# yyamamoto79/guetzli-cuda-opencl

Measured on AMD Instinct MI355X. Metric: Mpixels/s end-to-end encode @ q=95; achieved HBM GB/s on Butteraugli pass, higher is better.
Workload: dtype f32

## Files before the change

### guetzli-cuda-opencl_amd/csrc/kernels/gz_device.hip

```cpp
#include <hip/hip_runtime.h>

#include <math.h>
#include <stdio.h>
#include <string.h>
#include <time.h>

#include <algorithm>
#include <chrono>
#include <atomic>
#include <list>
#include <map>
#include <condition_variable>
#include <mutex>
#include <tuple>
#include <string>
#include <vector>

#include "../runtime/engine.h"
#include "../host/thread_pool.h"
#include "gz_math.h"

namespace gz {
__constant__ GzTables c_tab;
}
// ... 223 lines not shown
  do {                                                 \
    hipError_t e_ = (call);                            \
    if (e_ != hipSuccess) return Fail(#call, (int)e_); \
  } while (0)
#define GZ_LAUNCH()                                               \
  do {                                                            \
    hipError_t e_ = hipGetLastError();                            \
    if (e_ != hipSuccess) return Fail("kernel launch", (int)e_);  \
  } while (0)

namespace {
std::atomic<int> g_prof_on{0};
std::mutex g_prof_mu;
std::map<std::string, std::pair<long, double>> g_prof;
}

void ProfileEnable(bool on) { g_prof_on.store(on ? 1 : 0); }
void ProfileReset() {
  std::lock_guard<std::mutex> lk(g_prof_mu);
  g_prof.clear();
}
bool ProfileGet(const char* name, long* count, double* total_ms) {
  std::lock_guard<std::mutex> lk(g_prof_mu);
  auto it = g_prof.find(name);
  if (it == g_prof.end()) return false;
  *count = it->second.first;
  *total_ms = it->second.second;
  return true;
}
std::string ProfileNames() {
  std::lock_guard<std::mutex> lk(g_prof_mu);
  std::string out;
  for (auto& kv : g_prof) {
    if (!out.empty()) out += ",";
    out += kv.first;
  }
  return out;
}

void Engine::ProfBegin(const char* name) {
  if (!g_prof_on.load()) return;
  hipEvent_t a = nullptr, b = nullptr;
  if (hipEventCreate(&a) != hipSuccess || hipEventCreate(&b) != hipSuccess) return;
  hipEventRecord(a, static_cast<hipStream_t>(stream_));
  pending_.push_back({name, a, b});
}
void Engine::ProfEnd() {
  if (pending_.empty() || !g_prof_on.load()) return;
  hipEventRecord(static_cast<hipEvent_t>(pending_.back().stop), static_cast<hipStream_t>(stream_));
}
void Engine::ProfMark(const char* name) {
  if (!g_prof_on.load()) return;
  for (auto it = pending_.rbegin(); it != pending_.rend(); ++it)
    if (it->name == name) {
      hipEventRecord(static_cast<hipEvent_t>(it->stop), static_cast<hipStream_t>(stream_));
      return;
    }
}

void Engine::ProfFlush() {
  if (pending_.empty()) return;
  std::lock_guard<std::mutex> lk(g_prof_mu);
  for (auto& p : pending_) {
    float ms = 0.0f;
    if (hipEventSynchronize(static_cast<hipEvent_t>(p.stop)) == hipSuccess &&
        hipEventElapsedTime(&ms, static_cast<hipEvent_t>(p.start), static_cast<hipEvent_t>(p.stop)) == hipSuccess) {
      auto& e = g_prof[p.name];
      e.first += 1;
      e.second += ms;
    }
    hipEventDestroy(static_cast<hipEvent_t>(p.start));
    hipEventDestroy(static_cast<hipEvent_t>(p.stop));
  }
  pending_.clear();
}

#define GZ_TIMED(name, ...) \
  do {                      \
    ProfBegin(name);        \
    __VA_ARGS__;            \
    ProfEnd();              \
    GZ_LAUNCH();            \
  } while (0)

bool Engine::Fail(const char* what, int code) {
  char buf[256];
  snprintf(buf, sizeof(buf), "%s failed: %s (%d)", what,
           hipGetErrorString(static_cast<hipError_t>(code)), code);
  err_ = buf;
  failed_ = true;
  return false;
}

std::unique_ptr<Engine> Engine::Create(int device, int w, int h, std::string* err) {
  std::unique_ptr<Engine> e(new Engine);
  auto fail = [&](const std::string& m) {
    if (err) *err = m;
    return std::unique_ptr<Engine>();
  };
  if (w < 8 || h < 8 || w >= (1 << 16) || h >= (1 << 16)) return fail("unsupported image size");
  int ndev = 0;
  if (hipGetDeviceCount(&ndev) != hipSuccess || ndev == 0) return fail("no HIP device available");
  if (device < 0 || device >= ndev || device >= 64) return fail("bad device index");
  if (hipSetDevice(device) != hipSuccess) return fail("hipSetDevice failed");
  {
    std::lock_guard<std::mutex> lk(g_tab_mu);
    if (!g_tab_uploaded[device]) {
      const GzTables& t = HostTables();
      for (const BlurSpec& b : t.blur)
        if ((kBlurTile - 1) * b.step + 2 * b.radius + 1 + b.step > kBlurLds || 2 * b.radius + 1 > kMaxTaps ||
            b.step < 1 || b.step > 4)
          return fail("blur spec exceeds the tiled kernel's LDS span");
      for (int sig = 0; sig < kNumSigmas; ++sig)
        if (t.blur[sig].step != kBlurGeomStep[sig] || t.blur[sig].radius != kBlurGeomR[sig])
          return fail("blur geometry differs from the compiled BlurGeom table");
      for (int sig = kSigEdgeX; sig <= kSigEdgeB; ++sig)
        if (t.blur[sig].step != 1 || t.blur[sig].radius > kB2MaxR)
          return fail("edge blur spec does not fit the fused 2-D kernel");
      if (hipMemcpyToSymbol(HIP_SYMBOL(c_tab), &t, sizeof(t)) != hipSuccess)
        return fail("table upload failed");
      g_tab_uploaded[device] = true;
    }
  }
  e->device_ = device;
  e->w_ = w;
  e->h_ = h;
  e->bw_ = (w + 7) / 8;
  e->bh_ = (h + 7) / 8;
  e->nb_ = e->bw_ * e->bh_;
  e->rw_ = (w + 2) / 3;
  e->rh_ = (h + 2) / 3;
  e->n_ = static_cast<size_t>(w) * h;
  hipStream_t s;
  if (hipStreamCreateWithFlags(&s, hipStreamNonBlocking) != hipSuccess) return fail("stream");
  e->stream_ = s;
  const size_t n = e->n_, rn = static_cast<size_t>(e->rw_) * e->rh_;
  const size_t nc = static_cast<size_t>(e->nb_) * 64 * 3;
  bool ok = true;
  auto alloc = [&](void** p, size_t bytes) {
    if (ok && hipMalloc(p, bytes) != hipSuccess) ok = false;
    e->bytes_ += bytes;
  };
  alloc(reinterpret_cast<void**>(&e->d_rgb_), 3 * n);
  alloc(reinterpret_cast<void**>(&e->d_orig_), nc * sizeof(int16_t));
  alloc(reinterpret_cast<void**>(&e->d_cur_), nc * sizeof(int16_t));
  alloc(reinterpret_cast<void**>(&e->d_ref_xyb_), 3 * n * 4);
  alloc(reinterpret_cast<void**>(&e->d_lin_), 3 * n * 4);
  alloc(reinterpret_cast<void**>(&e->d_px8_), n * 4);
  alloc(reinterpret_cast<void**>(&e->d_xyb_), 3 * n * 4);
  alloc(reinterpret_cast<void**>(&e->d_m0_), 3 * n * 4);
  alloc(reinterpret_cast<void**>(&e->d_m1_), 3 * n * 4);
  alloc(reinterpret_cast<void**>(&e->d_tmp_), 6 * n * 4);
  alloc(reinterpret_cast<void**>(&e->d_bl_), 6 * n * 4);
  alloc(reinterpret_cast<void**>(&e->d_ma_), 3 * n * 4);
  alloc(reinterpret_cast<void**>(&e->d_mb_), 3 * n * 4);
  alloc(reinterpret_cast<void**>(&e->d_edge_), 3 * rn * 4);
  alloc(reinterpret_cast<void**>(&e->d_dc_), 3 * rn * 4);
  alloc(reinterpret_cast<void**>(&e->d_ac_), 3 * rn * 4);
  alloc(reinterpret_cast<void**>(&e->d_resval_), rn * 4);
  alloc(reinterpret_cast<void**>(&e->d_block_max_), e->nb_ * 4);
  alloc(reinterpret_cast<void**>(&e->d_mask_scale_), 3 * e->nb_ * 4);
  alloc(&e->d_zero_out_, static_cast<size_t>(e->nb_) * 192 * sizeof(CoeffData));
  alloc(reinterpret_cast<void**>(&e->d_zero_count_), static_cast<size_t>(e->nb_) * 4);
  alloc(reinterpret_cast<void**>(&e->d_zero_order_), static_cast<size_t>(e->nb_) * 4);
  alloc(reinterpret_cast<void**>(&e->d_zero_off_), static_cast<size_t>(e->nb_ + 1) * 4);
  alloc(reinterpret_cast<void**>(&e->d_zero_nnz_), static_cast<size_t>(e->nb_) * 4);
// ... 835 lines not shown
  }
  GZ_HIP(hipMemsetAsync(static_cast<char*>(d_ord_) + L.mbe, 0, static_cast<size_t>(nb_) * 4, s));
  GZ_HIP(hipMemsetAsync(static_cast<char*>(d_ord_) + L.sel, 0, L.cnt8 - L.sel, s));
  ord_adv_dir_ = 0;
  ord_n_ = 0;
  return true;
}

bool Engine::OrderEntriesCapacity(size_t n) {
  const size_t bytes = n * sizeof(OrderEntry);
  if (bytes > d_ord_entries_cap_) {
    if (d_ord_entries_) GZ_HIP(hipFree(d_ord_entries_));
    d_ord_entries_ = nullptr;
    d_ord_entries_cap_ = 0;
    const size_t cap = bytes + bytes / 4 + 4096;
    GZ_HIP(hipMalloc(&d_ord_entries_, cap));
    d_ord_entries_cap_ = cap;
  }
  return true;
}

bool Engine::OrderBuild(int direction, int rblock, double target_distance, bool zero_bmax,
                        const std::vector<int>& last_indexes, size_t* n_entries, int* blocks_to_change,
                        float floor_limit, int64_t* below_floor) {
  hipStream_t s = static_cast<hipStream_t>(stream_);
  GZ_HIP(hipSetDevice(device_));
  if (ord_cand_n_ < 0 || !d_ord_) return Fail("OrderBuild without candidates", 0);
  const size_t max_entries = static_cast<size_t>(ord_cand_n_) + static_cast<size_t>(nb_);
  if (!OrderEntriesCapacity(max_entries)) return false;
  if (static_cast<int>(last_indexes.size()) != nb_ || rblock < 1 || rblock > 4)
    return Fail("OrderBuild arguments", 0);
  const OrdLayout L(nb_);
  char* base = static_cast<char*>(d_ord_);
  uint32_t* sel = reinterpret_cast<uint32_t*>(base + L.sel);
  int adv_dir = 0;
  if (rblock == 1) {
    uint8_t* l8 = reinterpret_cast<uint8_t*>(h_ord_);
    int bad = 0;
    for (int b = 0; b < nb_; ++b) {
      bad |= last_indexes[b] & ~0xff;
      l8[b] = static_cast<uint8_t>(last_indexes[b]);
    }
    if (bad) return Fail("OrderBuild: last index above 255", 0);
    adv_dir = ord_adv_dir_;
    ord_adv_dir_ = 0;
  }
  ord_h1_ ^= 1;
  BuildArgs g;
  g.bmax = d_block_max_;
  g.zero_bmax = zero_bmax ? 1 : 0;
  g.bw = bw_;
  g.bh = bh_;
  g.r = rblock;
  g.direction = direction;
  g.td = target_distance;
  g.weight = reinterpret_cast<float*>(base + L.weight);
  g.active = reinterpret_cast<const int*>(base + L.active);
  g.mbe = reinterpret_cast<float*>(base + L.mbe);
  g.adv_vt = ord_adv_vt_;
  g.adv_dir = adv_dir;
  g.copy_last = rblock == 1 ? 1 : 0;
  g.last = reinterpret_cast<int*>(base + L.last);
  g.last_host = reinterpret_cast<const uint8_t*>(m_ord_);
  g.off = d_zero_off_;
  g.cand_n = ord_cand_n_;
  g.cand_err = d_cand_err_;
  g.out = static_cast<OrderEntry*>(d_ord_entries_);
  g.h1 = sel + SelLayout::h1 + ord_h1_ * kSelBins;
  g.h1_next = sel + SelLayout::h1 + (ord_h1_ ^ 1) * kSelBins;
  SelState* st = reinterpret_cast<SelState*>(sel + SelLayout::state);
  g.reserve = &st->reserve[ord_h1_];
  g.reserve_next = &st->reserve[ord_h1_ ^ 1];
  const unsigned groups = static_cast<unsigned>((nb_ + kBuildBlocks - 1) / kBuildBlocks);
  g.wg_host = m_ord_ + nb_ + kOrdInfoInts + 16 + static_cast<int>((sizeof(SelHost) + 63) / 64 * 16);
  const int* wg = h_ord_ + nb_ + kOrdInfoInts + 16 + static_cast<int>((sizeof(SelHost) + 63) / 64 * 16);
  g.floor_limit = floor_limit;
  g.blo = ord_lo_;
  g.bhi = std::min(ord_hi_, nb_);
  ord_h1_summed_ = false;
  if (direction < 0 && (rblock > 1 || !GZ_FUSE_ACTIVE))
    GZ_TIMED("order_build", k_order_active<<<static_cast<unsigned>((nb_ + 255) / 256), 256, 0, s>>>(
                                d_block_max_, zero_bmax ? 1 : 0, bw_, bh_, rblock, target_distance,
                                reinterpret_cast<int*>(base + L.active)));
  GZ_TIMED("order_build", k_order_build<<<groups, 256, 0, s>>>(g));
  GZ_HIP(WaitOnStream(s));
  ProfFlush();
  long long tot[3] = {0, 0, 0};
  for (unsigned k = 0; k < groups; ++k)
    for (int x = 0; x < 3; ++x) tot[x] += wg[4 * k + x];
  *blocks_to_change = static_cast<int>(tot[1]);
  *n_entries = static_cast<size_t>(tot[0]);
  if (below_floor) *below_floor = tot[2];
  ord_n_ = *n_entries;
  return true;
}

bool Engine::OrderFetch(std::pair<int, float>* out, size_t n) {
  static_assert(sizeof(OrderEntry) == sizeof(std::pair<int, float>), "entry layout");
  hipStream_t s = static_cast<hipStream_t>(stream_);
  GZ_HIP(hipSetDevice(device_));
  if (!n) return true;
  if (n != ord_n_) return Fail("OrderFetch entry count", 0);
  const size_t bytes = n * sizeof(OrderEntry);
  if (bytes > h_ord_entries_cap_) {
    if (h_ord_entries_) GZ_HIP(hipHostFree(h_ord_entries_));
    h_ord_entries_ = nullptr;
    h_ord_entries_cap_ = 0;
    const size_t cap = bytes + bytes / 4 + 4096;
    GZ_HIP(hipHostMalloc(&h_ord_entries_, cap));
    h_ord_entries_cap_ = cap;
  }
  GZ_HIP(hipMemcpyAsync(h_ord_entries_, d_ord_entries_, bytes, hipMemcpyDeviceToHost, s));
  GZ_HIP(WaitIdle(s));
  ProfFlush();
  const auto* src = static_cast<const std::pair<int, float>*>(h_ord_entries_);
  const int* wg = h_ord_ + nb_ + kOrdInfoInts + 16 + static_cast<int>((sizeof(SelHost) + 63) / 64 * 16);
  const int groups = (nb_ + kBuildBlocks - 1) / kBuildBlocks;
  size_t at = 0;
  for (int g = 0; g < groups; ++g) {
    const int cnt = wg[4 * g], base = wg[4 * g + 3];
    if (cnt == 0) continue;
    if (cnt < 0 || base < 0 || static_cast<size_t>(base) + cnt > n || at + cnt > n)
      return Fail("OrderFetch: workgroup ranges", 0);
    memcpy(static_cast<void*>(out + at), src + base, static_cast<size_t>(cnt) * sizeof(OrderEntry));
    at += static_cast<size_t>(cnt);
  }
  if (at != n) return Fail("OrderFetch: entry count", 0);
  return true;
}

bool Engine::BulkCountsStaging() {
  if (h_bulk_) return true;
  void* h = nullptr;
  void* m = nullptr;
  if (hipHostMalloc(&h, static_cast<size_t>(nb_) + 64, hipHostMallocCoherent) != hipSuccess) {
    return Fail("BulkApply: pinned allocation failed", 0);
  }
  if (hipHostGetDevicePointer(&m, h, 0) != hipSuccess) {
    (void)hipHostFree(h);
    return Fail("BulkApply: mapped address", 0);
  }
  h_bulk_ = static_cast<uint8_t*>(h);
  m_bulk_ = static_cast<uint8_t*>(m);
  bytes_ += static_cast<size_t>(nb_) + 64;
  return true;
}

bool Engine::BulkApplyEnqueue(int direction, const int quant[3][64], const uint8_t* cnt_dev, const uint32_t* sel,
                              const uint8_t* last8, uint8_t* cnt_host) {
  hipStream_t s = static_cast<hipStream_t>(stream_);
  const OrdLayout L(nb_);
  QuantMatrix qm;
  memcpy(qm.q, quant, sizeof(qm.q));
  JpegQuantF qf;
  for (int c = 0; c < 3; ++c)
    for (int k = 0; k < 64; ++k) qf.qz[c][k] = static_cast<float>(quant[c][c_natural_order[k]]);
  const size_t stage_groups = (3 * static_cast<size_t>(nb_) + kStageBlocks - 1) / kStageBlocks;
  const unsigned groups = static_cast<unsigned>(
      std::min(stage_groups, (static_cast<size_t>(nb_) + kBulkWaves - 1) / kBulkWaves));
  GZ_TIMED("bulk_apply", k_bulk_apply<<<groups, kBulkThreads, 0, s>>>(
      cnt_dev, reinterpret_cast<const int*>(static_cast<char*>(d_ord_) + L.last), d_zero_off_, ord_cand_n_,
      d_cand_idx_, nb_, direction, d_orig_, qm, qf, d_cur_, d_jhist_, sel, last8, cnt_host),
      k_hist_fold<<<1, 1024, 0, s>>>(d_jhist_, m_jhist_, 0));
  return true;
}

bool Engine::BulkApply(int direction, const int quant[3][64], const uint8_t* cnt, int32_t delta[3][256],
                       const std::vector<int>* last_indexes) {
  hipStream_t s = static_cast<hipStream_t>(stream_);
  GZ_HIP(hipSetDevice(device_));
  if (last_indexes && !d_ord_ && !OrderReset()) return false;
  if (ord_cand_n_ < 0 || !d_ord_) return Fail("BulkApply without a change order", 0);
  if (!BulkCountsStaging()) return false;
  memcpy(h_bulk_, cnt, static_cast<size_t>(nb_));
  const uint8_t* last8 = nullptr;
  if (last_indexes) {
    if (static_cast<int>(last_indexes->size()) != nb_) return Fail("BulkApply: last indexes", 0);
    uint8_t* l8 = reinterpret_cast<uint8_t*>(h_ord_);
    int bad = 0;
    for (int b = 0; b < nb_; ++b) {
      bad |= (*last_indexes)[b] & ~0xff;
      l8[b] = static_cast<uint8_t>((*last_indexes)[b]);
    }
    if (bad) return Fail("BulkApply: last index above 255", 0);
    last8 = reinterpret_cast<const uint8_t*>(m_ord_);
  }
  if (!BulkApplyEnqueue(direction, quant, m_bulk_, nullptr, last8, nullptr)) return false;
  GZ_HIP(WaitOnStream(s));
  ProfFlush();
  for (int c = 0; c < 3; ++c)
    for (int i = 0; i < 256; ++i) delta[c][i] = static_cast<int32_t>(h_jhist_[(2 * c + 1) * 256 + i]);
  return true;
}

static size_t SelCollectLds(int cap) {
  return 2 * static_cast<size_t>(cap) * sizeof(unsigned long long) + (kSelSortBins + 1) * sizeof(uint32_t);
}

bool Engine::OrderSelect(size_t bulk, size_t window, int direction, const int quant[3][64], bool apply,
                         OrderSelection* out, int32_t delta[3][256]) {
  hipStream_t s = static_cast<hipStream_t>(stream_);
  GZ_HIP(hipSetDevice(device_));
  if (ord_cand_n_ < 0 || !d_ord_) return Fail("OrderSelect without a change order", 0);
  const size_t n = ord_n_;
  if ((ord_x_ ? ord_frame_n_ : n) == 0 || bulk >= (ord_x_ ? ord_frame_n_ : n) || window == 0)
    return Fail("OrderSelect arguments", 0);
  if (!BulkCountsStaging()) return false;
  window = std::min<size_t>(window, kSelCandMax / 2);
  if (!h_win_) {
    GZ_HIP(hipHostMalloc(&h_win_, kSelCandMax * sizeof(OrderEntry), hipHostMallocCoherent));
    GZ_HIP(hipHostGetDevicePointer(&m_win_, h_win_, 0));
    GZ_HIP(hipMalloc(&d_win_, kSelCandMax * sizeof(unsigned long long)));
    bytes_ += kSelCandMax * sizeof(unsigned long long);
    GZ_HIP(hipFuncSetAttribute(reinterpret_cast<const void*>(k_sel_finish),
                               hipFuncAttributeMaxDynamicSharedMemorySize,
                               static_cast<int>(SelCollectLds(kSelCandMax))));
  }
  int cap = 1024;
  while (static_cast<size_t>(cap) < 2 * window && cap < kSelCandMax) cap <<= 1;
  const OrdLayout L(nb_);
  char* base = static_cast<char*>(d_ord_);
  uint32_t* sel = reinterpret_cast<uint32_t*>(base + L.sel);
  uint8_t* cnt8 = reinterpret_cast<uint8_t*>(base + L.cnt8);
  const OrderEntry* e = static_cast<const OrderEntry*>(d_ord_entries_);
  const int has_prefix = bulk > 0 ? 1 : 0;
  const size_t fn = ord_x_ ? ord_frame_n_ : n;
  const long long ta = static_cast<long long>(bulk) - 1;
  const long long tb = static_cast<long long>(std::min(fn - 1, bulk + window - 1));
  SelHost* host = reinterpret_cast<SelHost*>(h_ord_ + nb_ + kOrdInfoInts + 16);
  SelHost* mhost = reinterpret_cast<SelHost*>(m_ord_ + nb_ + kOrdInfoInts + 16);
  host->done = 0;
  static const int force_open = getenv("GZ_SELECT_OPEN") ? atoi(getenv("GZ_SELECT_OPEN")) : 0;
  const size_t chunks = (n + 1023) / 1024;
  const unsigned rgroups = static_cast<unsigned>(std::max<size_t>(1, std::min<size_t>(512, chunks)));
  static const size_t cmax = getenv("GZ_SEL_CGROUPS") ? static_cast<size_t>(atoi(getenv("GZ_SEL_CGROUPS"))) : 512;
  const unsigned cgroups = static_cast<unsigned>(std::max<size_t>(1, std::min<size_t>(cmax, chunks)));
  uint32_t* h1 = sel + SelLayout::h1 + ord_h1_ * kSelBins;
  const int blo = ord_x_ ? ord_lo_ : 0, bhi = ord_x_ ? std::min(ord_hi_, nb_) : nb_;
  const int gbase = ord_x_ ? ord_gbase_ : 0;
  if (!ord_x_) {
    GZ_TIMED("order_select",
             (k_sel_refine<<<rgroups, 256, 0, s>>>(e, static_cast<int>(n), has_prefix, ta, tb, h1, sel,
                                                    reinterpret_cast<uint32_t*>(cnt8), (nb_ + 3) / 4),
              k_sel_collect<<<cgroups, kSelThreads, 0, s>>>(e, static_cast<int>(n), has_prefix,
                                                             static_cast<long long>(bulk), ta, tb, sel,
                                                             reinterpret_cast<uint32_t*>(cnt8),
// ... 344 lines not shown
```

### guetzli-cuda-opencl_amd/csrc/kernels/jpeg_kernels.inc

```
#pragma once

namespace gz {

struct JpegQuantF {
  float qz[3][64];
};

constexpr int kJDcSyms = 17;
struct JpegCodesArg {
  uint8_t dc[3][kJDcSyms][3];
  uint8_t ac[3][256][3];
};

constexpr int c_natural_order[64] = {
    0,  1,  8,  16, 9,  2,  3,  10, 17, 24, 32, 25, 18, 11, 4,  5,  12, 19, 26, 33, 40, 48,
    41, 34, 27, 20, 13, 6,  7,  14, 21, 28, 35, 42, 49, 56, 57, 50, 43, 36, 29, 22, 15, 23,
    30, 37, 44, 51, 58, 59, 52, 45, 38, 31, 39, 46, 53, 60, 61, 54, 47, 55, 62, 63,
};

__device__ __forceinline__ int log2_floor_nz(uint32_t v) { return 31 - __clz(v); }

__device__ __forceinline__ int16_t jpeg_quant(int16_t v, float q) {
  return static_cast<int16_t>(static_cast<int>(static_cast<float>(v) / q));
}

__device__ __forceinline__ int16_t jpeg_quant_rcp(int16_t v, int q, float rq) {
  const int a = v < 0 ? -static_cast<int>(v) : static_cast<int>(v);
  int n = static_cast<int>(static_cast<float>(a) * rq);
  n -= n * q > a ? 1 : 0;
  n += (n + 1) * q <= a ? 1 : 0;
  return static_cast<int16_t>(v < 0 ? -n : n);
}

__device__ __forceinline__ int16_t jpeg_dc(const int16_t* __restrict__ cur, const JpegQuantF& q,
                                           int nb, int c, int b) {
  if (b < 0) return 0;
  return jpeg_quant(cur[(static_cast<size_t>(c) * nb + b) * 64], q.qz[c][0]);
}

constexpr int kJHistCopies = 8;
__global__ __launch_bounds__(1024) void k_hist_fold(uint32_t* __restrict__ hist, uint32_t* __restrict__ host_out,
                                                    int chroma) {
  for (int i = threadIdx.x; i < 6 * 256; i += 1024) {
    uint32_t v = 0;
#pragma unroll
    for (int k = 0; k < kJHistCopies; ++k) {
      v += hist[k * (6 * 256) + i];
      hist[k * (6 * 256) + i] = 0u;
    }
    host_out[i] = v;
  }
  if (chroma && threadIdx.x == 0) {
    unsigned long long* chroma_nz = reinterpret_cast<unsigned long long*>(hist + kJHistCopies * 6 * 256);
    unsigned long long cn = 0;
    for (int k = 0; k < kJHistCopies; ++k) {
      cn += chroma_nz[k];
      chroma_nz[k] = 0ull;
    }
    host_out[6 * 256] = static_cast<uint32_t>(cn);
    host_out[6 * 256 + 1] = static_cast<uint32_t>(cn >> 32);
  }
}
__host__ __device__ constexpr size_t jhist_device_bytes(size_t stage_groups) {
  return kJHistCopies * 6 * 256 * 4 + kJHistCopies * 8 + (2 + stage_groups / 64 + 1) * 4;
}
constexpr int kStageBlocks = 256;
constexpr int kStageThreads = 4 * kStageBlocks;
constexpr int kStageStride = 33;

template <int kQuarter>
__device__ __forceinline__ void jpeg_stage_quarter(const uint32_t* __restrict__ sb, int c,
                                                   const JpegQuantF& q, int16_t z[16], uint32_t* m16,
                                                   int* nz_stored) {
  const int16_t* v = reinterpret_cast<const int16_t*>(sb);
  uint32_t m = 0;
  int nz = 0;
#pragma unroll
  for (int i = 0; i < 16; ++i) {
    const int k = 16 * kQuarter + i;
    const int16_t sv = v[c_natural_order[k]];
    nz += sv != 0;
    z[i] = jpeg_quant(sv, q.qz[c][k]);
    m |= static_cast<uint32_t>(z[i] != 0) << i;
  }
  *m16 = m;
  *nz_stored = nz;
}

template <int kQuarter>
__device__ __forceinline__ void jpeg_stage_symbols(const int16_t z[16], uint64_t m64,
                                                   uint32_t* __restrict__ hac) {
#pragma unroll
  for (int i = 0; i < 16; ++i) {
    const int k = 16 * kQuarter + i;
    if (k == 0 || z[i] == 0) continue;
    const uint64_t below = m64 & ~1ull & ((1ull << k) - 1);
    const int prev = below ? 63 - __clzll(below) : 0;
    const int run = k - prev - 1;
    if (run > 15) atomicAdd(&hac[0xf0], static_cast<uint32_t>(run >> 4));
    const int a = z[i] < 0 ? -z[i] : z[i];
    atomicAdd(&hac[((run & 15) << 4) + log2_floor_nz(a) + 1], 1u);
  }
}

__global__ __launch_bounds__(kStageThreads) void k_jpeg_stage(const int16_t* __restrict__ cur, JpegQuantF q,
                                                     int nb, int m0, int m1,
                                                     uint32_t* __restrict__ hist) {
  unsigned long long* chroma_nz = reinterpret_cast<unsigned long long*>(hist + kJHistCopies * 6 * 256);
  __shared__ uint32_t lh_all[4][6 * 256];
  __shared__ uint32_t sblk[kStageBlocks * kStageStride];
  __shared__ uint16_t smask[kStageBlocks][4];
  __shared__ int nz_red[kStageThreads / 64];
  const int tid = threadIdx.x, lane = tid & 63, wv = tid >> 6;
  for (int i = tid; i < 4 * 6 * 256; i += kStageThreads) (&lh_all[0][0])[i] = 0;
  const int nr = m1 - m0;
  const int ntot = 3 * nr;
  const int t0 = blockIdx.x * kStageBlocks;
  {
#pragma unroll
    for (int r = 0; r < 2; ++r) {
      const int j = tid + kStageThreads * r;
      const int lb = j >> 3, part = j & 7;
      if (t0 + lb < ntot) {
        const int tt = t0 + lb, cc = tt / nr;
        const uint4 u = reinterpret_cast<const uint4*>(
            cur + (static_cast<size_t>(cc) * nb + m0 + (tt - cc * nr)) * 64)[part];
        uint32_t* d = &sblk[lb * kStageStride + 4 * part];
        d[0] = u.x;
        d[1] = u.y;
        d[2] = u.z;
        d[3] = u.w;
      }
    }
  }
  __syncthreads();
  const int quarter = wv & 3;
  const int lb = 64 * (wv >> 2) + lane;
  const bool on = t0 + lb < ntot;
  const int c = on ? (t0 + lb) / nr : 0;
  const int t = c * nb + m0 + (t0 + lb - c * nr);
  int16_t z[16];
  uint32_t m16 = 0;
  int nz_stored = 0;
  if (on) {
// ... 435 lines not shown
      s_tail = v;
    } else {
      words[fw + i - wbase] = v;
      ff += count_ff_bytes(v, nbytes);
    }
  }
  ff = wave_sum_i(ff);
  if (lane == 0) s_ff[wv] = ff;
  __syncthreads();
  if (tid == 0) {
    int f = s_ff[0] + s_ff[1] + s_ff[2] + s_ff[3];
    const bool one = nw == 1;
    if (head_shared) {
      if (t == 0) {
        host[kCodeHostFirst] = s_head;
      } else {
        const uint64_t info = (one && tail_shared) ? 8u : static_cast<uint64_t>(one ? end_bytes : 4);
        code_store(&side[2 * t], (info << 32) | s_head);
        asm volatile("s_waitcnt vmcnt(0)" ::: "memory");
        if (atomicAdd(&seam[t], 1u) == 1u) {
          asm volatile("" ::: "memory");
          atomicExch(&seam[t], 0u);
          const uint32_t v = static_cast<uint32_t>(code_load(&side[2 * t - 1])) | s_head;
          if (info & 8u) {
            host[kCodeHostLast] = v;
          } else {
            words[fw - wbase] = v;
            f += count_ff_bytes(v, static_cast<int>(info));
          }
        }
      }
    }
    if (tail_shared && !(one && head_shared)) {
      if (last_wg) {
        host[kCodeHostLast] = s_tail;
      } else {
        code_store(&side[2 * t + 1], static_cast<uint64_t>(s_tail));
        asm volatile("s_waitcnt vmcnt(0)" ::: "memory");
        if (atomicAdd(&seam[t + 1], 1u) == 1u) {
          asm volatile("" ::: "memory");
          atomicExch(&seam[t + 1], 0u);
          const uint64_t h = code_load(&side[2 * (t + 1)]);
          const uint32_t v = static_cast<uint32_t>(h) | s_tail;
          const uint32_t info = static_cast<uint32_t>(h >> 32);
          if (info & 8u) {
            host[kCodeHostLast] = v;
          } else {
            words[lwd - wbase] = v;
            f += count_ff_bytes(v, static_cast<int>(info));
          }
        }
      }
    }
    host[kCodeHostFf + t] = static_cast<uint32_t>(f);
    if (last_wg) {
      const unsigned long long total = E - base;
      host[kCodeHostBits] = static_cast<uint32_t>(total);
      host[kCodeHostBits + 1] = static_cast<uint32_t>(total >> 32);
    }
  }
}


constexpr int kBulkThreads = 1024;
constexpr int kBulkWaves = kBulkThreads / 64;

__device__ __forceinline__ void bulk_symbols(int16_t z, int lane, uint32_t* h, uint32_t w) {
  const uint64_t m = __ballot(z != 0) & ~1ull;
  if (lane > 0 && z != 0) {
    const uint64_t below = m & ((1ull << lane) - 1);
    const int prev = below ? 63 - __clzll(below) : 0;
    const int run = lane - prev - 1;
    if (run > 15) atomicAdd(&h[0xf0], w * static_cast<uint32_t>(run >> 4));
    const int a = z < 0 ? -z : z;
    atomicAdd(&h[((run & 15) << 4) + log2_floor_nz(a) + 1], w);
  }
  if (lane == 63 && !(m >> 63)) atomicAdd(&h[0], w);
}

__global__ __launch_bounds__(kBulkThreads) void k_bulk_apply(
    const uint8_t* __restrict__ cnt, const int* __restrict__ last, const int* __restrict__ off, int cand_n,
    const uint8_t* __restrict__ cand_idx, int nb, int direction, const int16_t* __restrict__ orig,
    const QuantMatrix qm, const JpegQuantF q, int16_t* __restrict__ cur, uint32_t* __restrict__ hist,
    const uint32_t* __restrict__ sel, const uint8_t* __restrict__ last8, uint8_t* __restrict__ cnt_host) {
  if (sel && reinterpret_cast<const SelState*>(sel + SelLayout::state)->open) return;
  __shared__ uint32_t lh[3 * 256];
  __shared__ float lq[3 * 64];
  __shared__ int lqm[3 * 64];
  __shared__ uint8_t lchg[kBulkWaves][3 * 64];
  const int tid = threadIdx.x, lane = tid & 63, wv = wave_id();
  for (int i = tid; i < 3 * 256; i += kBulkThreads) lh[i] = 0;
  if (tid < 3 * 64) {
    lq[tid] = reinterpret_cast<const float*>(&q)[tid];
    lqm[tid] = reinterpret_cast<const int*>(&qm)[tid];
  }
  __syncthreads();
  const int nat = c_natural_order[lane];
  uint8_t* chg = lchg[wv];
  const int back = direction < 0 ? -1 : 0;
  const int nw = static_cast<int>(gridDim.x) * kBulkWaves;
  const int w = static_cast<int>(blockIdx.x) * kBulkWaves + wv;
  for (int b0 = w; b0 < nb; b0 += 64 * nw) {
    const int bl = b0 + lane * nw;
    const int my_n = bl < nb ? cnt[bl] : 0;
    if (cnt_host && bl < nb) cnt_host[bl] = static_cast<uint8_t>(my_n);
    const int my_off = my_n ? max(0, min(off[bl], cand_n - 1)) : 0;
    const int my_li = my_n ? (last8 ? static_cast<int>(last8[bl]) : last[bl]) : 0;
    uint64_t todo = __ballot(my_n != 0);
    while (todo) {
      const int j = __builtin_ctzll(todo);
      todo &= todo - 1;
      const int b = b0 + j * nw;
      const int n = __builtin_amdgcn_readlane(my_n, j);
      const int first = __builtin_amdgcn_readlane(my_off, j) + __builtin_amdgcn_readlane(my_li, j) + back;
      int16_t v[3];
#pragma unroll
      for (int c = 0; c < 3; ++c) v[c] = cur[(static_cast<size_t>(c) * nb + b) * 64 + nat];
      int ci[3];
#pragma unroll
      for (int r = 0; r < 3; ++r) ci[r] = lane + 64 * r < n ? cand_idx[first + (lane + 64 * r) * direction] : -1;
      chg[lane] = 0;
      chg[64 + lane] = 0;
      chg[128 + lane] = 0;
      asm volatile("s_waitcnt lgkmcnt(0)" ::: "memory");
#pragma unroll
      for (int r = 0; r < 3; ++r)
        if (ci[r] >= 0) chg[ci[r]] = 1;
      asm volatile("s_waitcnt lgkmcnt(0)" ::: "memory");
#pragma unroll
      for (int c = 0; c < 3; ++c) {
        const bool ch = chg[64 * c + nat] != 0;
        if (!__ballot(ch)) continue;
        const size_t e = (static_cast<size_t>(c) * nb + b) * 64 + nat;
        int16_t nv = v[c];
        if (ch) {
          nv = direction > 0 ? static_cast<int16_t>(0) : quantize_coeff(orig[e], lqm[64 * c + nat]);
          cur[e] = nv;
        }
        const float qq = lq[64 * c + lane];
        const int16_t z0 = jpeg_quant(v[c], qq), z1 = jpeg_quant(nv, qq);
        if (!__ballot(z0 != z1)) continue;
        bulk_symbols(z0, lane, &lh[256 * c], ~0u);
        bulk_symbols(z1, lane, &lh[256 * c], 1u);
      }
    }
  }
  __syncthreads();
  uint32_t* hcopy = hist + (blockIdx.x % kJHistCopies) * (6 * 256);
  for (int i = tid; i < 3 * 256; i += kBulkThreads) {
    const uint32_t v = lh[i];
    if (v) atomicAdd(&hcopy[(2 * (i >> 8) + 1) * 256 + (i & 255)], v);
  }
}

}
```

### guetzli-cuda-opencl_amd/csrc/kernels/order_kernels.inc

```
#pragma once

namespace gz {

__device__ __forceinline__ float order_max(float a, float b) { return a < b ? b : a; }

__device__ __forceinline__ void order_range(const int* __restrict__ off, int cand_n, int b, int* offset,
                                            int* num) {
  *offset = max(0, min(off[b], cand_n - 1));
  *num = off[b + 1] - *offset;
}

__device__ __forceinline__ float order_local_max(const float* __restrict__ bmax, int zero_bmax, int bw, int bh,
                                                 int bx, int by, int r, float tdf) {
  float m = tdf;
  for (int y = max(0, by - r); y < min(bh, by + 1 + r); ++y) {
    float rm = tdf;
    for (int x = max(0, bx - r); x < min(bw, bx + 1 + r); ++x) rm = order_max(rm, zero_bmax ? 0.0f : bmax[y * bw + x]);
    m = order_max(m, rm);
  }
  return m;
}
__global__ __launch_bounds__(256) void k_order_active(const float* __restrict__ bmax, int zero_bmax, int bw, int bh,
                                                      int r, double td, int* __restrict__ active) {
  const int b = blockIdx.x * 256 + threadIdx.x;
// ... 51 lines not shown
  const int t = threadIdx.x, lane = t & 63, wv = t >> 6;
  uint32_t v[2][per];
  int loc[2] = {0, 0};
#pragma unroll
  for (int x = 0; x < 2; ++x) {
    const uint4* p = reinterpret_cast<const uint4*>((x ? hb : ha) + t * per);
#pragma unroll
    for (int q = 0; q < per / 4; ++q) {
      const uint4 u = p[q];
      v[x][4 * q] = u.x;
      v[x][4 * q + 1] = u.y;
      v[x][4 * q + 2] = u.z;
      v[x][4 * q + 3] = u.w;
    }
#pragma unroll
    for (int k = 0; k < per; ++k) loc[x] += static_cast<int>(v[x][k]);
  }
  int inc[2] = {loc[0], loc[1]};
#pragma unroll
  for (int d = 1; d < 64; d <<= 1) {
#pragma unroll
    for (int x = 0; x < 2; ++x) {
      const int o = __shfl_up(inc[x], d, 64);
      if (lane >= d) inc[x] += o;
    }
  }
  if (lane == 63) {
    s_w[0][wv] = inc[0];
    s_w[1][wv] = inc[1];
  }
  if (t == 0) {
    s_res.j[0] = kSelBins - 1;
    s_res.below[0] = base_a;
    s_res.eq[0] = 0;
    s_res.j[1] = kSelBins - 1;
    s_res.below[1] = base_b;
    s_res.eq[1] = 0;
  }
  __syncthreads();
#pragma unroll
  for (int x = 0; x < 2; ++x) {
    if (x == 0 && !want_a) continue;
    int pre = 0;
    for (int k = 0; k < wv; ++k) pre += s_w[x][k];
    const long long target = x ? tb : ta;
    long long cum = static_cast<long long>(x ? base_b : base_a) + pre + inc[x] - loc[x];
    const bool last = t == NT - 1;
    if ((cum <= target && cum + loc[x] > target) || (last && cum + loc[x] <= target)) {
      int j = t * per + per - 1;
      int eq = static_cast<int>(v[x][per - 1]);
      long long below = cum + loc[x] - eq;
#pragma unroll
      for (int k = 0; k < per; ++k) {
        if (cum + v[x][k] > target) {
          j = t * per + k;
          below = cum;
          eq = static_cast<int>(v[x][k]);
          break;
        }
        cum += v[x][k];
      }
      s_res.j[x] = j;
      s_res.below[x] = static_cast<int>(below);
      s_res.eq[x] = eq;
    }
  }
  __syncthreads();
  *res = s_res;
  __syncthreads();
}

struct OrderEntry {
  int block;
  float key;
};
#ifndef GZ_FUSE_ACTIVE
#define GZ_FUSE_ACTIVE 1
#endif
#ifndef GZ_BUILD_BLOCKS
#define GZ_BUILD_BLOCKS 128
#endif
constexpr int kBuildBlocks = GZ_BUILD_BLOCKS;
static_assert(kBuildBlocks <= 256 && 256 % kBuildBlocks == 0, "blocks per build workgroup");
struct BuildArgs {
  const float* bmax;
  int zero_bmax, bw, bh, r, direction;
  double td;
  float* weight;
  const int* active;
  float* mbe;
  float adv_vt;
  int adv_dir;
  int copy_last;
  int* last;
  const uint8_t* last_host;
  const int* off;
  int cand_n;
  const float* cand_err;
  OrderEntry* out;
  uint32_t* h1;
  uint32_t* h1_next;
  int* reserve;
  int* reserve_next;
  int* wg_host;
  float floor_limit;
  int blo, bhi;
};
__global__ __launch_bounds__(256) void k_order_build(BuildArgs g) {
  __shared__ int s_off[256 + 1];
  __shared__ int s_last[kBuildBlocks], s_cand[kBuildBlocks];
  __shared__ float s_w[kBuildBlocks], s_mbe[kBuildBlocks];
  __shared__ uint32_t s_h[kSelBins];
  __shared__ int s_base, s_with, s_below;
  __shared__ int s_wsum[4], s_wwith[4];
  const int t = threadIdx.x, lane = t & 63, wv = t >> 6;
  const int nb = g.bw * g.bh;
  const int b0 = static_cast<int>(blockIdx.x) * kBuildBlocks;
  for (int k = static_cast<int>(blockIdx.x) * 256 + t; k < kSelBins; k += static_cast<int>(gridDim.x) * 256)
    g.h1_next[k] = 0u;
  if (blockIdx.x == 0 && t == 0) *g.reserve_next = 0;
  if (t == 0) s_below = 0;
  const int b = b0 + t;
  int e = 0;
  if (t < kBuildBlocks && b < nb) {
    const int bx = b % g.bw, by = b / g.bw;
    const int li = g.copy_last ? static_cast<int>(g.last_host[b]) : g.last[b];
    const int off0 = g.off[b], off1 = g.off[b + 1];
    float mbe = g.mbe[b];
    const float wold = g.adv_dir ? g.weight[b] : 0.0f;
    float w = 0.0f;
    if (g.r == 1) {
      const int xs[3] = {max(bx - 1, 0), bx, min(bx + 1, g.bw - 1)};
      const int ys[3] = {max(by - 1, 0), by, min(by + 1, g.bh - 1)};
      const bool xin[3] = {bx > 0, true, bx + 1 < g.bw}, yin[3] = {by > 0, true, by + 1 < g.bh};
      if (g.direction > 0) {
        float v[3][3];
#pragma unroll
        for (int i = 0; i < 3; ++i)
#pragma unroll
          for (int j = 0; j < 3; ++j) v[i][j] = g.zero_bmax ? 0.0f : g.bmax[ys[i] * g.bw + xs[j]];
        const float tdf = static_cast<float>(g.td);
        float m = tdf;
#pragma unroll
        for (int i = 0; i < 3; ++i) {
          if (!yin[i]) continue;
          float rm = tdf;
#pragma unroll
          for (int j = 0; j < 3; ++j)
            if (xin[j]) rm = order_max(rm, v[i][j]);
          m = order_max(m, rm);
        }
        const float mine = v[1][1];
        w = (static_cast<double>(mine) <= g.td && static_cast<double>(m) <= 1.1 * g.td) ? 1.0f : 0.0f;
      } else {
        int d = 2;
#if GZ_FUSE_ACTIVE
        float v5[5][5];
        bool y5[5], x5[5];
#pragma unroll
        for (int i = 0; i < 5; ++i) {
          y5[i] = by - 2 + i >= 0 && by - 2 + i < g.bh;
          x5[i] = bx - 2 + i >= 0 && bx - 2 + i < g.bw;
        }
#pragma unroll
        for (int i = 0; i < 5; ++i) {
          const int yc = min(max(by - 2 + i, 0), g.bh - 1);
#pragma unroll
          for (int j = 0; j < 5; ++j) {
            const int xc = min(max(bx - 2 + j, 0), g.bw - 1);
            v5[i][j] = g.zero_bmax ? 0.0f : g.bmax[yc * g.bw + xc];
          }
        }
        const float tdf = static_cast<float>(g.td);
        constexpr double kLocalMaxWeight = 0.5;
#pragma unroll
        for (int i = 0; i < 3; ++i)
#pragma unroll
          for (int j = 0; j < 3; ++j) {
            if (!(yin[i] && xin[j])) continue;
            float m = tdf;
#pragma unroll
            for (int di = 0; di < 3; ++di) {
              if (!y5[i + di]) continue;
              float rm = tdf;
#pragma unroll
              for (int dj = 0; dj < 3; ++dj)
                if (x5[j + dj]) rm = order_max(rm, v5[i + di][j + dj]);
              m = order_max(m, rm);
            }
            const float mine = v5[i + 1][j + 1];
            const bool act = !(static_cast<double>(mine) <=
                               (1 - kLocalMaxWeight) * g.td + kLocalMaxWeight * static_cast<double>(m));
            if (act) d = min(d, (i == 1 && j == 1) ? 0 : 1);
          }
#else
        int a[3][3];
#pragma unroll
        for (int i = 0; i < 3; ++i)
#pragma unroll
          for (int j = 0; j < 3; ++j) a[i][j] = g.active[ys[i] * g.bw + xs[j]];
#pragma unroll
        for (int i = 0; i < 3; ++i)
#pragma unroll
          for (int j = 0; j < 3; ++j)
            if (yin[i] && xin[j] && a[i][j]) d = min(d, (i == 1 && j == 1) ? 0 : 1);
#endif
        w = d <= 1 ? 1.0f / (d + 1.0f) : 0.0f;
      }
    } else if (g.direction > 0) {
      const float m = order_local_max(g.bmax, g.zero_bmax, g.bw, g.bh, bx, by, g.r, static_cast<float>(g.td));
      const float mine = g.zero_bmax ? 0.0f : g.bmax[b];
      w = (static_cast<double>(mine) <= g.td && static_cast<double>(m) <= 1.1 * g.td) ? 1.0f : 0.0f;
    } else {
      int d = g.r + 1;
      for (int y = max(0, by - g.r); y < min(g.bh, by + 1 + g.r); ++y)
        for (int x = max(0, bx - g.r); x < min(g.bw, bx + 1 + g.r); ++x)
          if (g.active[y * g.bw + x]) d = min(d, max(abs(x - bx), abs(y - by)));
      w = d <= g.r ? 1.0f / (d + 1.0f) : 0.0f;
    }
    if (g.adv_dir) {
      mbe += wold * g.adv_vt * g.adv_dir;
      g.mbe[b] = mbe;
    }
    if (g.copy_last) g.last[b] = li;
    g.weight[b] = w;
    const int offset = max(0, min(off0, g.cand_n - 1));
    const int num = off1 - offset;
    if (w != 0.0f && b >= g.blo && b < g.bhi) e = g.direction > 0 ? max(0, num - li) : li;
    s_w[t] = w;
    s_mbe[t] = mbe;
    s_last[t] = li;
    s_cand[t] = offset;
  }
  int inc = e;
#pragma unroll
  for (int d = 1; d < 64; d <<= 1) {
    const int o = __shfl_up(inc, d, 64);
    if (lane >= d) inc += o;
  }
  const int with = static_cast<int>(__popcll(__ballot(e > 0)));
  if (lane == 63) {
    s_wsum[wv] = inc;
    s_wwith[wv] = with;
  }
  __syncthreads();
  int pre = 0;
  for (int k = 0; k < wv; ++k) pre += s_wsum[k];
  s_off[t + 1] = pre + inc;
  if (t == 0) s_off[0] = 0;
  if (t == 255) {
    const int tot = pre + inc;
    s_base = tot ? atomicAdd(g.reserve, tot) : 0;
    s_with = s_wwith[0] + s_wwith[1] + s_wwith[2] + s_wwith[3];
  }
  __syncthreads();
  const int total = s_off[256], base = s_base;
  const bool lds_hist = total > 0;
  if (lds_hist) {
    for (int k = t; k < kSelBins; k += 256) s_h[k] = 0u;
    __syncthreads();
  }
  for (int k0 = 0; k0 < total; k0 += 256) {
    const int k = k0 + t;
    const bool valid = k < total;
    float key = 0.0f;
    if (valid) {
      int lo = 0, hi = kBuildBlocks;
      while (hi - lo > 1) {
        const int mid = (lo + hi) >> 1;
        if (s_off[mid] <= k) lo = mid; else hi = mid;
      }
      const int j = k - s_off[lo];
      const float* errs = g.cand_err + s_cand[lo];
      key = g.direction > 0 ? (errs[s_last[lo] + j] - s_mbe[lo]) / s_w[lo]
                            : (s_mbe[lo] - errs[s_last[lo] - 1 - j]) / s_w[lo];
      g.out[base + k] = OrderEntry{b0 + lo, key};
      atomicAdd(&s_h[order_bits(key) >> 20], 1u);
    }
    const uint64_t below = __ballot(valid && key < g.floor_limit);
    if (lane == 0 && below) atomicAdd(&s_below, static_cast<int>(__popcll(below)));
  }
  __syncthreads();
  if (lds_hist)
    for (int k = t; k < kSelBins; k += 256)
      if (s_h[k]) atomicAdd(&g.h1[k], s_h[k]);
  if (t == 0) {
    int* o = g.wg_host + 4 * blockIdx.x;
    o[0] = total;
    o[1] = s_with;
    o[2] = s_below;
    o[3] = base;
  }
}

constexpr int kSelSortBins = 4096;
constexpr int kSelBucketMax = 96;
template <int E>
__device__ void sel_order(unsigned long long* __restrict__ sk, unsigned long long* __restrict__ tmp,
                          uint32_t* __restrict__ hist, const unsigned long long* __restrict__ cand, int nc,
                          uint32_t lo24, uint32_t hi24) {
  __shared__ int s_w[kSelThreads / 64];
  __shared__ int s_big;
  const int t = threadIdx.x, lane = t & 63, wv = t >> 6;
  int sh = 0;
  while (((hi24 - lo24) >> sh) >= static_cast<uint32_t>(kSelSortBins)) ++sh;
  for (int k = t; k < kSelSortBins; k += kSelThreads) hist[k] = 0u;
  unsigned long long v[E];
  int bin[E], slot[E];
#pragma unroll
  for (int e = 0; e < E; ++e) {
    const int i = t * E + e;
    v[e] = i < nc ? cand[i] : 0ull;
    bin[e] = static_cast<int>(((static_cast<uint32_t>(v[e] >> 40)) - lo24) >> sh);
  }
  __syncthreads();
#pragma unroll
  for (int e = 0; e < E; ++e)
    if (t * E + e < nc) slot[e] = static_cast<int>(atomicAdd(&hist[bin[e]], 1u));
  __syncthreads();
  constexpr int per = kSelSortBins / kSelThreads;
  uint32_t c[per];
  int loc = 0, big = 0;
#pragma unroll
  for (int k = 0; k < per; ++k) {
    c[k] = hist[t * per + k];
    loc += static_cast<int>(c[k]);
    big |= c[k] > static_cast<uint32_t>(kSelBucketMax) ? 1 : 0;
  }
  int inc = loc;
#pragma unroll
  for (int d = 1; d < 64; d <<= 1) {
    const int o = __shfl_up(inc, d, 64);
    if (lane >= d) inc += o;
  }
  if (lane == 63) s_w[wv] = inc;
  if (t == 0) s_big = 0;
  __syncthreads();
  if (big) s_big = 1;
  __syncthreads();
  if (s_big) {
    int n2 = 2;
    while (n2 < nc) n2 <<= 1;
#pragma unroll
    for (int e = 0; e < E; ++e)
      if (t * E + e < nc) sk[t * E + e] = v[e];
    for (int i = nc + t; i < n2; i += kSelThreads) sk[i] = ~0ull;
    __syncthreads();
    for (int size = 2; size <= n2; size <<= 1)
      for (int stride = size >> 1; stride > 0; stride >>= 1) {
        for (int q = t; q < n2 / 2; q += kSelThreads) {
          const int i = 2 * q - (q & (stride - 1));
          const int j = i + stride;
          const bool up = (i & size) == 0;
          const unsigned long long x = sk[i], y = sk[j];
          if ((x > y) == up) {
            sk[i] = y;
            sk[j] = x;
          }
        }
        __syncthreads();
      }
    return;
  }
  int run = inc - loc;
  for (int k = 0; k < wv; ++k) run += s_w[k];
#pragma unroll
  for (int k = 0; k < per; ++k) {
// ... 225 lines not shown
```

Measured before the change: 292.8.

## Fuse histogram fold into bulk_apply last block and widen order_build workgroups

Adds a last-block-arrives pattern to k_bulk_apply: an atomic arrival counter picks the final workgroup, which folds the per-copy histograms into host memory and clears them. This removes the separate k_hist_fold launch, with an env/macro toggle to turn it off. Separately, k_order_build now launches with 1024 threads (default) instead of 256, so the entry-emission and LDS histogram clear loops are spread over more threads, while the prefix scan is kept to the first 256 threads. The risks are memory-ordering correctness of the cross-block fold and extra wasted threads in the scan phase.

```diff
diff --git a/guetzli-cuda-opencl_amd/csrc/kernels/gz_device.hip b/guetzli-cuda-opencl_amd/csrc/kernels/gz_device.hip
--- a/guetzli-cuda-opencl_amd/csrc/kernels/gz_device.hip
+++ b/guetzli-cuda-opencl_amd/csrc/kernels/gz_device.hip
@@ -329,6 +329,11 @@
     ProfEnd();              \
     GZ_LAUNCH();            \
   } while (0)
+
+static bool FuseFold() {
+  static const bool on = getenv("GZ_FUSE_FOLD") ? atoi(getenv("GZ_FUSE_FOLD")) != 0 : GZ_FUSE_FOLD != 0;
+  return on;
+}
 
 bool Engine::Fail(const char* what, int code) {
   char buf[256];
@@ -1330,7 +1335,7 @@
     GZ_TIMED("order_build", k_order_active<<<static_cast<unsigned>((nb_ + 255) / 256), 256, 0, s>>>(
                                 d_block_max_, zero_bmax ? 1 : 0, bw_, bh_, rblock, target_distance,
                                 reinterpret_cast<int*>(base + L.active)));
-  GZ_TIMED("order_build", k_order_build<<<groups, 256, 0, s>>>(g));
+  GZ_TIMED("order_build", k_order_build<<<groups, kBuildThreads, 0, s>>>(g));
   GZ_HIP(WaitOnStream(s));
   ProfFlush();
   long long tot[3] = {0, 0, 0};
@@ -1408,8 +1413,9 @@
       std::min(stage_groups, (static_cast<size_t>(nb_) + kBulkWaves - 1) / kBulkWaves));
   GZ_TIMED("bulk_apply", k_bulk_apply<<<groups, kBulkThreads, 0, s>>>(
       cnt_dev, reinterpret_cast<const int*>(static_cast<char*>(d_ord_) + L.last), d_zero_off_, ord_cand_n_,
-      d_cand_idx_, nb_, direction, d_orig_, qm, qf, d_cur_, d_jhist_, sel, last8, cnt_host),
-      k_hist_fold<<<1, 1024, 0, s>>>(d_jhist_, m_jhist_, 0));
+      d_cand_idx_, nb_, direction, d_orig_, qm, qf, d_cur_, d_jhist_, sel, last8, cnt_host,
+      FuseFold() ? m_jhist_ : nullptr),
+      FuseFold() ? (void)0 : k_hist_fold<<<1, 1024, 0, s>>>(d_jhist_, m_jhist_, 0));
   return true;
 }
 
diff --git a/guetzli-cuda-opencl_amd/csrc/kernels/jpeg_kernels.inc b/guetzli-cuda-opencl_amd/csrc/kernels/jpeg_kernels.inc
--- a/guetzli-cuda-opencl_amd/csrc/kernels/jpeg_kernels.inc
+++ b/guetzli-cuda-opencl_amd/csrc/kernels/jpeg_kernels.inc
@@ -60,6 +60,44 @@
     host_out[6 * 256] = static_cast<uint32_t>(cn);
     host_out[6 * 256 + 1] = static_cast<uint32_t>(cn >> 32);
   }
+}
+#ifndef GZ_FUSE_FOLD
+#define GZ_FUSE_FOLD 1
+#endif
+template <int NT>
+__device__ __forceinline__ void hist_fold_last(uint32_t* __restrict__ hist, uint32_t* __restrict__ host_out) {
+  __shared__ int s_fold_last;
+  const int tid = threadIdx.x;
+  asm volatile("s_waitcnt vmcnt(0)" ::: "memory");
+  __syncthreads();
+  uint32_t* arrived = hist + kJHistCopies * 6 * 256 + kJHistCopies * 2;
+  if (tid == 0)
+    s_fold_last = __hip_atomic_fetch_add(arrived, 1u, __ATOMIC_RELAXED, __HIP_MEMORY_SCOPE_AGENT) ==
+                  static_cast<uint32_t>(gridDim.x) - 1u;
+  __syncthreads();
+  if (!s_fold_last) return;
+  constexpr int kIt = (6 * 256 + NT - 1) / NT;
+  uint32_t c[kIt][kJHistCopies];
+#pragma unroll
+  for (int it = 0; it < kIt; ++it) {
+    const int i = min(tid + NT * it, 6 * 256 - 1);
+#pragma unroll
+    for (int k = 0; k < kJHistCopies; ++k)
+      c[it][k] = __hip_atomic_load(&hist[k * (6 * 256) + i], __ATOMIC_RELAXED, __HIP_MEMORY_SCOPE_AGENT);
+  }
+#pragma unroll
+  for (int it = 0; it < kIt; ++it) {
+    const int i = tid + NT * it;
+    if (i >= 6 * 256) break;
+    uint32_t v = 0;
+#pragma unroll
+    for (int k = 0; k < kJHistCopies; ++k) {
+      v += c[it][k];
+      if (c[it][k]) __hip_atomic_store(&hist[k * (6 * 256) + i], 0u, __ATOMIC_RELAXED, __HIP_MEMORY_SCOPE_AGENT);
+    }
+    host_out[i] = v;
+  }
+  if (tid == 0) __hip_atomic_store(arrived, 0u, __ATOMIC_RELAXED, __HIP_MEMORY_SCOPE_AGENT);
 }
 __host__ __device__ constexpr size_t jhist_device_bytes(size_t stage_groups) {
   return kJHistCopies * 6 * 256 * 4 + kJHistCopies * 8 + (2 + stage_groups / 64 + 1) * 4;
@@ -661,8 +699,13 @@
     const uint8_t* __restrict__ cnt, const int* __restrict__ last, const int* __restrict__ off, int cand_n,
     const uint8_t* __restrict__ cand_idx, int nb, int direction, const int16_t* __restrict__ orig,
     const QuantMatrix qm, const JpegQuantF q, int16_t* __restrict__ cur, uint32_t* __restrict__ hist,
-    const uint32_t* __restrict__ sel, const uint8_t* __restrict__ last8, uint8_t* __restrict__ cnt_host) {
-  if (sel && reinterpret_cast<const SelState*>(sel + SelLayout::state)->open) return;
+    const uint32_t* __restrict__ sel, const uint8_t* __restrict__ last8, uint8_t* __restrict__ cnt_host,
+    uint32_t* __restrict__ fold_out) {
+  if (sel && reinterpret_cast<const SelState*>(sel + SelLayout::state)->open) {
+    if (fold_out && blockIdx.x == 0)
+      for (int i = threadIdx.x; i < 6 * 256; i += kBulkThreads) fold_out[i] = 0u;
+    return;
+  }
   __shared__ uint32_t lh[3 * 256];
   __shared__ float lq[3 * 64];
   __shared__ int lqm[3 * 64];
@@ -730,6 +773,7 @@
     const uint32_t v = lh[i];
     if (v) atomicAdd(&hcopy[(2 * (i >> 8) + 1) * 256 + (i & 255)], v);
   }
-}
-
-}
+  if (fold_out) hist_fold_last<kBulkThreads>(hist, fold_out);
+}
+
+}
diff --git a/guetzli-cuda-opencl_amd/csrc/kernels/order_kernels.inc b/guetzli-cuda-opencl_amd/csrc/kernels/order_kernels.inc
--- a/guetzli-cuda-opencl_amd/csrc/kernels/order_kernels.inc
+++ b/guetzli-cuda-opencl_amd/csrc/kernels/order_kernels.inc
@@ -157,6 +157,11 @@
 #endif
 constexpr int kBuildBlocks = GZ_BUILD_BLOCKS;
 static_assert(kBuildBlocks <= 256 && 256 % kBuildBlocks == 0, "blocks per build workgroup");
+#ifndef GZ_BUILD_THREADS
+#define GZ_BUILD_THREADS 1024
+#endif
+constexpr int kBuildThreads = GZ_BUILD_THREADS;
+static_assert(kBuildThreads >= 256 && kBuildThreads <= 1024 && kBuildThreads % 256 == 0, "build workgroup");
 struct BuildArgs {
   const float* bmax;
   int zero_bmax, bw, bh, r, direction;
@@ -181,7 +186,7 @@
   float floor_limit;
   int blo, bhi;
 };
-__global__ __launch_bounds__(256) void k_order_build(BuildArgs g) {
+__global__ __launch_bounds__(kBuildThreads) void k_order_build(BuildArgs g) {
   __shared__ int s_off[256 + 1];
   __shared__ int s_last[kBuildBlocks], s_cand[kBuildBlocks];
   __shared__ float s_w[kBuildBlocks], s_mbe[kBuildBlocks];
@@ -191,7 +196,8 @@
   const int t = threadIdx.x, lane = t & 63, wv = t >> 6;
   const int nb = g.bw * g.bh;
   const int b0 = static_cast<int>(blockIdx.x) * kBuildBlocks;
-  for (int k = static_cast<int>(blockIdx.x) * 256 + t; k < kSelBins; k += static_cast<int>(gridDim.x) * 256)
+  for (int k = static_cast<int>(blockIdx.x) * kBuildThreads + t; k < kSelBins;
+       k += static_cast<int>(gridDim.x) * kBuildThreads)
     g.h1_next[k] = 0u;
   if (blockIdx.x == 0 && t == 0) *g.reserve_next = 0;
   if (t == 0) s_below = 0;
@@ -314,14 +320,14 @@
     if (lane >= d) inc += o;
   }
   const int with = static_cast<int>(__popcll(__ballot(e > 0)));
-  if (lane == 63) {
+  if (lane == 63 && wv < 4) {
     s_wsum[wv] = inc;
     s_wwith[wv] = with;
   }
   __syncthreads();
   int pre = 0;
-  for (int k = 0; k < wv; ++k) pre += s_wsum[k];
-  s_off[t + 1] = pre + inc;
+  for (int k = 0; k < min(wv, 4); ++k) pre += s_wsum[k];
+  if (t < 256) s_off[t + 1] = pre + inc;
   if (t == 0) s_off[0] = 0;
   if (t == 255) {
     const int tot = pre + inc;
@@ -332,10 +338,10 @@
   const int total = s_off[256], base = s_base;
   const bool lds_hist = total > 0;
   if (lds_hist) {
-    for (int k = t; k < kSelBins; k += 256) s_h[k] = 0u;
+    for (int k = t; k < kSelBins; k += kBuildThreads) s_h[k] = 0u;
     __syncthreads();
   }
-  for (int k0 = 0; k0 < total; k0 += 256) {
+  for (int k0 = 0; k0 < total; k0 += kBuildThreads) {
     const int k = k0 + t;
     const bool valid = k < total;
     float key = 0.0f;
@@ -357,7 +363,7 @@
   }
   __syncthreads();
   if (lds_hist)
-    for (int k = t; k < kSelBins; k += 256)
+    for (int k = t; k < kSelBins; k += kBuildThreads)
       if (s_h[k]) atomicAdd(&g.h1[k], s_h[k]);
   if (t == 0) {
     int* o = g.wg_host + 4 * blockIdx.x;
```

New measurement: 159.2. 45.6% lower.
